# TortillasAlfred/NeuralBarkCalculator

Hardware: NVIDIA B200
Metric: images/sec (higher is better)
Workload: dtype fp16

## Files before the change

include/nbc.h:

```cpp
#ifndef NBC_H_
#define NBC_H_

#include <stddef.h>
#include <stdint.h>

#ifdef __cplusplus
extern "C" {
#endif

typedef enum {
  NBC_OK = 0,
  NBC_ERR_INVALID = -1,
  NBC_ERR_CUDA = -2,
  NBC_ERR_DEVICE = -3,
  NBC_ERR_WORKSPACE = -4,
  NBC_ERR_KERNEL = -5
} nbc_status;

typedef struct nbc_plan nbc_plan;

int nbc_version(void);
const char* nbc_last_error(void);
int nbc_device_check(int device);
int64_t nbc_launch_count(void);
// ... 15 lines not shown
                size_t workspace_bytes, void* stream);

int nbc_fold_bn_pack(const float* w, const float* gamma, const float* beta, const float* mean, const float* var,
                     const float* conv_bias, float eps, int Cout, int Cin, int kh, int kw, int cin_pad, int f16,
                     void* w_packed_bf16, float* bias_out, void* stream);

typedef struct {
  int32_t N, H, W, Cin, Cout;
  int32_t kh, kw, stride, pad, dil;
  int32_t relu;
  int32_t impl;
  int32_t f16;
} nbc_conv_desc;
int nbc_conv_bf16(const nbc_conv_desc* desc, const void* x, const void* w_packed, const float* bias,
                  const void* residual, void* y, void* stream);

int nbc_conv_dual_bf16(const nbc_conv_desc* desc, const void* x, const nbc_conv_desc* desc2, const void* x2,
                       const void* w_cat, const float* bias, void* y, void* stream);

int nbc_conv_wgrad_bf16(const nbc_conv_desc* desc, const void* dz, const void* x, float* dw, void* stream);

int nbc_stem_u8(const uint8_t* img, int N, int H, int W, const float* mean3_host, const float* std3_host,
                const float* w_stem, const float* bias, void* out, void* stream);
int nbc_stem_f32(const float* x_nchw, int N, int H, int W, const float* w_stem, const float* bias, void* out,
                 void* stream);
size_t nbc_stem_tc_workspace_bytes(int N, int H, int W);
int nbc_stem_pack_weights(const float* w_stem_f32, int f16, void* w224_bf16, void* stream);
int nbc_stem_tc(const void* input, int input_kind, int N, int H, int W, const float* mean3_host,
                const float* std3_host, const void* w224_bf16, const float* bias, int f16, void* workspace,
                size_t workspace_bytes, void* out, void* stream);
// ... 106 lines not shown
```

neuralbarkcalculator_b200/_lib.py:

```python
import ctypes as C
import os

_HERE = os.path.dirname(os.path.abspath(__file__))
LIB_PATH = os.path.join(_HERE, 'libnbc.so')

c_void_p, c_int, c_i64, c_size_t, c_float = C.c_void_p, C.c_int, C.c_int64, C.c_size_t, C.c_float


class ConvDesc(C.Structure):
    _fields_ = [(n, C.c_int32) for n in ('N', 'H', 'W', 'Cin', 'Cout', 'kh', 'kw', 'stride', 'pad', 'dil', 'relu', 'impl', 'f16')]


class PlanStep(C.Structure):
    _fields_ = ([('name', C.c_char * 24)]
                + [(n, C.c_int32) for n in ('kind', 'pair', 'halo3', 'stem_halo', 'dual', 'block_n', 'kblk', 'out_bufs',
                                            'ragged_map', 'N', 'H', 'W', 'Cin', 'Cout', 'k', 'stride', 'pad', 'dil', 'relu',
                                            'H2', 'W2', 'Cin2', 'stride2', 'level')]
                + [(n, C.c_int64) for n in ('x', 'x2', 'residual', 'y', 'levels')])


SIGNATURES = {
    'nbc_version': (c_int, []),
    'nbc_last_error': (C.c_char_p, []),
    'nbc_device_check': (c_int, [c_int]),
    'nbc_launch_count': (c_i64, []),
    'nbc_preprocess_workspace_bytes': (c_size_t, [c_int, c_int]),
    'nbc_preprocess_4x_u8': (c_int, [c_void_p, c_int, c_int, c_i64, c_int, c_void_p, c_void_p, c_void_p, c_size_t, c_void_p]),
    'nbc_preprocess_4x_span_u8': (c_int, [c_void_p, c_int, c_int, c_i64, c_int, c_int, c_int, c_void_p, c_void_p, c_void_p, c_size_t,
                                          c_void_p]),
    'nbc_preprocess_4x_batch_u8': (c_int, [c_void_p, c_void_p, c_void_p, c_int, c_int, c_int, c_i64, c_int, c_void_p, c_i64, c_void_p,
                                           c_void_p, c_size_t, c_void_p]),
    'nbc_host_zero_row_span': (c_int, [c_void_p, c_int, c_i64, c_i64, c_int, c_void_p, c_void_p]),
    'nbc_preprocess_general_workspace_bytes': (c_size_t, [c_int, c_int, c_int]),
    'nbc_preprocess_general_u8': (c_int, [c_void_p, c_int, c_int, c_i64, c_int, c_int, c_void_p, c_void_p, c_void_p, c_size_t,
                                  c_void_p]),
    'nbc_trim_u8': (c_int, [c_void_p, c_int, c_int, c_void_p, c_void_p, c_void_p, c_size_t, c_void_p]),
    'nbc_fold_bn_pack': (c_int, [c_void_p] * 6 + [c_float, c_int, c_int, c_int, c_int, c_int, c_int, c_void_p, c_void_p, c_void_p]),
    'nbc_conv_bf16': (c_int, [C.POINTER(ConvDesc), c_void_p, c_void_p, c_void_p, c_void_p, c_void_p, c_void_p]),
    'nbc_conv_dual_bf16': (c_int, [C.POINTER(ConvDesc), c_void_p, C.POINTER(ConvDesc), c_void_p, c_void_p, c_void_p, c_void_p, c_void_p]),
    'nbc_conv_wgrad_bf16': (c_int, [C.POINTER(ConvDesc), c_void_p, c_void_p, c_void_p, c_void_p]),
    'nbc_stem_u8': (c_int, [c_void_p, c_int, c_int, c_int, C.POINTER(c_float), C.POINTER(c_float), c_void_p, c_void_p, c_void_p, c_void_p]),
    'nbc_stem_f32': (c_int, [c_void_p, c_int, c_int, c_int, c_void_p, c_void_p, c_void_p, c_void_p]),
    'nbc_stem_tc_workspace_bytes': (c_size_t, [c_int, c_int, c_int]),
    'nbc_stem_pack_weights': (c_int, [c_void_p, c_int, c_void_p, c_void_p]),
    'nbc_stem_tc': (c_int, [c_void_p, c_int, c_int, c_int, c_int, C.POINTER(c_float), C.POINTER(c_float), c_void_p, c_void_p,
                    c_int, c_void_p, c_size_t, c_void_p, c_void_p]),
    'nbc_maxpool3x3s2_bf16': (c_int, [c_void_p, c_int, c_int, c_int, c_int, c_int, c_void_p, c_void_p]),
    'nbc_head_1x1': (c_int, [c_void_p, c_i64, c_int, c_int, c_int, c_void_p, c_void_p, c_void_p, c_void_p]),
    'nbc_upsample_argmax': (c_int, [c_void_p, c_int, c_int, c_int, c_int, c_int, c_void_p, c_void_p]),
    'nbc_upsample_bicubic': (c_int, [c_void_p, c_int, c_int, c_int, c_int, c_int, c_int, c_void_p, c_void_p]),
    'nbc_upsample_argmax_ragged': (c_int, [c_void_p, c_int, c_int, c_int, c_int, c_int, c_void_p, c_void_p, c_void_p]),
    'nbc_heights_from_first_last': (c_int, [c_void_p, c_int, c_void_p, c_void_p]),
    'nbc_ccl_workspace_bytes': (c_size_t, [c_int, c_int, c_int]),
# ... 90 lines not shown
```

neuralbarkcalculator_b200/csrc/api.cu:

```cuda
#include <stdarg.h>

#include "common.cuh"
#include "conv.h"
#include "train.h"

namespace nbc {

static thread_local char g_err[1024] = "";
std::atomic<int64_t> g_launches{0};

void set_error(const char* fmt, ...) {
  va_list ap;
  va_start(ap, fmt);
  vsnprintf(g_err, sizeof(g_err), fmt, ap);
  va_end(ap);
}

int sm_count() {
  static int cached = 0;
  if (cached) return cached;
  int dev = 0, n = 0;
  if (cudaGetDevice(&dev) == cudaSuccess &&
      cudaDeviceGetAttribute(&n, cudaDevAttrMultiProcessorCount, dev) == cudaSuccess && n > 0)
    cached = n;
// ... 103 lines not shown
  NBC_REQUIRE((gamma != nullptr) == (beta != nullptr) && (gamma != nullptr) == (mean != nullptr) &&
                  (gamma != nullptr) == (var != nullptr),
              "nbc_fold_bn_pack: gamma/beta/mean/var must be all given or all NULL");
  NBC_REQUIRE(Cout > 0 && Cin > 0 && kh > 0 && kw > 0 && cin_pad >= Cin, "nbc_fold_bn_pack: bad shape");
  return fold_pack(w, gamma, beta, mean, var, conv_bias, eps, Cout, Cin, kh, kw, cin_pad, w_packed_bf16, nullptr,
                   bias_out, reinterpret_cast<cudaStream_t>(stream), f16 ? 1 : 0);
}

extern "C" int nbc_conv_bf16(const nbc_conv_desc* d, const void* x, const void* w_packed, const float* bias,
                             const void* residual, void* y, void* stream_) {
  cudaStream_t stream = reinterpret_cast<cudaStream_t>(stream_);
  NBC_REQUIRE(d && x && w_packed && bias && y, "nbc_conv_bf16: null pointer");
  ConvGeom g{d->N, d->H, d->W, d->Cin, d->Cout, d->kh, d->kw, d->stride, d->pad, d->dil, d->relu, d->f16 ? 1 : 0};
  NBC_REQUIRE(g.N > 0 && g.H > 0 && g.W > 0 && g.Ho() > 0 && g.Wo() > 0, "nbc_conv_bf16: bad shape");
  const bool tc_ok = conv_tc_supported(g);
  if (d->impl == 1 || (d->impl == 0 && tc_ok)) return conv_tc(g, x, w_packed, bias, residual, y, stream);
  if (d->impl == 2 || d->impl == 0) return conv_mma(g, x, w_packed, bias, residual, y, stream);
  set_error("nbc_conv_bf16: unknown impl %d", d->impl);
  return NBC_ERR_INVALID;
}

extern "C" int nbc_conv_wgrad_bf16(const nbc_conv_desc* d, const void* dz, const void* x, float* dw, void* stream_) {
  cudaStream_t stream = reinterpret_cast<cudaStream_t>(stream_);
  NBC_REQUIRE(d && dz && x && dw, "nbc_conv_wgrad_bf16: null pointer");
  NBC_REQUIRE(!d->f16, "nbc_conv_wgrad_bf16: the training path is bf16 only");
  ConvGeom g{d->N, d->H, d->W, d->Cin, d->Cout, d->kh, d->kw, d->stride, d->pad, d->dil, 0, 0};
  NBC_REQUIRE(g.N > 0 && g.H > 0 && g.W > 0 && g.Ho() > 0 && g.Wo() > 0, "nbc_conv_wgrad_bf16: bad shape");
  const bool tc_ok = wgrad_tc_supported(g);
  if (d->impl == 1 || (d->impl == 0 && tc_ok)) return wgrad_tc(g, dz, x, dw, stream);
  if (d->impl == 2 || d->impl == 0) return wgrad_mma(g, dz, x, dw, stream);
  set_error("nbc_conv_wgrad_bf16: unknown impl %d", d->impl);
  return NBC_ERR_INVALID;
}

// ... 12 lines not shown
```

neuralbarkcalculator_b200/csrc/common.cuh:

```cuda
#pragma once
#include <cuda.h>
#include <cuda_bf16.h>
#include <cuda_fp16.h>
#include <cuda_runtime.h>
#include <stdint.h>
#include <stdio.h>

#include <atomic>
#include <string>

#include "../../include/nbc.h"

namespace nbc {

void set_error(const char* fmt, ...);
extern std::atomic<int64_t> g_launches;
inline void count_launch(int n = 1) { g_launches.fetch_add(n, std::memory_order_relaxed); }

#define NBC_CUDA(expr)                                                                       \
  do {                                                                                       \
    cudaError_t _e = (expr);                                                                 \
    if (_e != cudaSuccess) {                                                                 \
      nbc::set_error("%s failed: %s (%s:%d)", #expr, cudaGetErrorString(_e), __FILE__, __LINE__); \
      return NBC_ERR_CUDA;                                                                   \
// ... 89 lines not shown
}
__device__ __forceinline__ void tma_load_2d(void* smem, const CUtensorMap* m, uint64_t* bar, int c0, int c1) {
  asm volatile(
      "cp.async.bulk.tensor.2d.shared::cluster.global.mbarrier::complete_tx::bytes [%0], [%1, {%3, %4}], [%2];" ::"r"(
          smem_u32(smem)),
      "l"(reinterpret_cast<uint64_t>(m)), "r"(smem_u32(bar)), "r"(c0), "r"(c1)
      : "memory");
}
__device__ __forceinline__ void tma_load_4d(void* smem, const CUtensorMap* m, uint64_t* bar, int c0, int c1, int c2,
                                            int c3) {
  asm volatile(
      "cp.async.bulk.tensor.4d.shared::cluster.global.mbarrier::complete_tx::bytes [%0], [%1, {%3, %4, %5, %6}], "
      "[%2];" ::"r"(smem_u32(smem)),
      "l"(reinterpret_cast<uint64_t>(m)), "r"(smem_u32(bar)), "r"(c0), "r"(c1), "r"(c2), "r"(c3)
      : "memory");
}

__device__ __forceinline__ void tma_store_4d(const CUtensorMap* m, const void* smem, int c0, int c1, int c2, int c3) {
  asm volatile("cp.async.bulk.tensor.4d.global.shared::cta.bulk_group [%0, {%2, %3, %4, %5}], [%1];" ::"l"(
                   reinterpret_cast<uint64_t>(m)),
               "r"(smem_u32(smem)), "r"(c0), "r"(c1), "r"(c2), "r"(c3)
               : "memory");
}
__device__ __forceinline__ void tma_store_commit() { asm volatile("cp.async.bulk.commit_group;" ::: "memory"); }
template <int N>
__device__ __forceinline__ void tma_store_wait_read() {
  asm volatile("cp.async.bulk.wait_group.read %0;" ::"n"(N) : "memory");
}
__device__ __forceinline__ void tma_store_wait_all() { asm volatile("cp.async.bulk.wait_group 0;" ::: "memory"); }

// ... 156 lines not shown
```

neuralbarkcalculator_b200/csrc/conv.h:

```cpp
#pragma once
#include <cuda_runtime.h>
#include <limits.h>
#include <stdint.h>
#include <string.h>

namespace nbc {

struct ConvGeom {
  int N, H, W, Cin, Cout;
  int kh, kw, stride, pad, dil;
  int relu;
  int f16 = 0;
  int Ho() const { return (H + 2 * pad - dil * (kh - 1) - 1) / stride + 1; }
  int Wo() const { return (W + 2 * pad - dil * (kw - 1) - 1) / stride + 1; }
  double flops() const { return 2.0 * N * Ho() * Wo() * (double)Cout * Cin * kh * kw; }
};

struct ConvTcPrepared {
  alignas(64) unsigned char storage[1536];
};
bool conv_tc_supported(const ConvGeom& g);
int conv_tc_prepare(const ConvGeom& g, const void* x, const void* w, const float* bias, const void* residual, void* y,
                    ConvTcPrepared* out, const int* valid_h = nullptr);
int conv_tc_prepare_dual(const ConvGeom& g, const void* x, const ConvGeom& g2, const void* x2, const void* w_cat,
                         const float* bias, void* y, ConvTcPrepared* out, const int* valid_h = nullptr);
int conv_tc_run(const ConvTcPrepared* prep, cudaStream_t stream);
struct ConvTcVariant {
  int pair, halo3, stem_halo, dual, block_n, kblk, out_bufs;
  int ragged_map;
};
void conv_tc_describe(const ConvTcPrepared* prep, ConvTcVariant* v);
int conv_tc_prepare_stem(int N, int Ho, int Wo, int Hp, int Wp, const void* padded, const void* w224, const float* bias,
                         void* y, ConvTcPrepared* out, const int* valid_h = nullptr, int f16 = 0, int relu = 1);
int conv_tc(const ConvGeom& g, const void* x, const void* w, const float* bias, const void* residual, void* y,
            cudaStream_t stream);

bool conv_mma_supported(const ConvGeom& g);
int conv_mma(const ConvGeom& g, const void* x, const void* w, const float* bias, const void* residual, void* y,
             cudaStream_t stream);

int stem_tc_pad(const void* input, int input_kind, int N, int H, int W, const float* mean3, const float* std3, void* padded,
                cudaStream_t stream, const int* valid_h, int f16 = 0);
int maxpool_ragged(const void* x, int N, int H, int W, int C, void* y, const int* valid_h, cudaStream_t stream,
                   int f16 = 0);
int head_1x1(const void* x16, int64_t pixels_per_image, int N, int Cin, const float* w3xC, const float* bias3,
             float* logits_planar, int f16, cudaStream_t stream, const int* valid_h = nullptr, int row_w = 1);
int ragged_levels(const int* heights, const int* first_last, int N, int Hc, int* levels, cudaStream_t stream);

int fold_pack(const float* w, const float* gamma, const float* beta, const float* mean, const float* var,
              const float* cb, float eps, int Cout, int Cin, int kh, int kw, int cin_pad, void* wp_bf16, float* wp_f32,
// ... 6 lines not shown
```

neuralbarkcalculator_b200/csrc/conv_tc.cu:

```cuda
#include "common.cuh"
#include "conv.h"

namespace nbc {

struct ConvTcParams {
  CUtensorMap tmA[4];
  CUtensorMap tmB;
  CUtensorMap tmOut;
  CUtensorMap tmRes;
  const float* bias;
  const __nv_bfloat16* residual;
  __nv_bfloat16* out;
  int N, Ho, Wo, Cout;
  int tw_log2, th, tw, tiles_w, tiles_h;
  int num_m_tiles, num_n_tiles;
  int n_taps, cblocks;
  int cblocks2, map2;
  int relu;
  int f16;
  const int* valid_h;
  int8_t tap_map[9];
  int16_t tap_dh[9];
  int16_t tap_dw[9];
  const uint8_t* stem_src;
// ... 547 lines not shown
    }
    __syncwarp();
  } else if (warp == 10) {
    output_role<BN, OB, RES>(p, s, walk);
  } else {
    epilogue_role<BN, OB, RES, RELU, F16>(p, s, walk);
  }
  tc_teardown<Cfg>(warp, s.tmem_base);
}

constexpr int kStemRowBytes = 2112;
constexpr int kStemStageBytes = 7 * kStemRowBytes + 64;
using StemCfg = TcLayout<6, kStemStageBytes, 7 * 64 * 64 , 64, 4, false>;
static_assert(StemCfg::kUsedBytes > 120 * 1024, "stem halo kernel: shared memory budget");

__device__ __forceinline__ void bulk_load_1d(void* smem, const void* gmem, uint32_t bytes, uint64_t* bar) {
  asm volatile("cp.async.bulk.shared::cluster.global.mbarrier::complete_tx::bytes [%0], [%1], %2, [%3];" ::"r"(smem_u32(smem)),
               "l"(reinterpret_cast<uint64_t>(gmem)), "r"(bytes), "r"(smem_u32(bar))
               : "memory");
}
__device__ __forceinline__ uint64_t umma_desc_kmajor_noswizzle(uint32_t smem_addr, uint32_t lbo_bytes, uint32_t sbo_bytes) {
  uint64_t d = 0;
  d |= (uint64_t)((smem_addr & 0x3FFFF) >> 4);
  d |= (uint64_t)(lbo_bytes >> 4) << 16;
  d |= (uint64_t)(sbo_bytes >> 4) << 32;
  d |= (uint64_t)1 << 46;
  return d;
}

template <bool RELU, bool F16>
__global__ void __launch_bounds__(kTcThreads, 1) conv_tc_stem_kernel(const __grid_constant__ ConvTcParams p) {
  using Cfg = StemCfg;
  constexpr int BN = 64;
  const int warp = __shfl_sync(0xffffffffu, (int)(threadIdx.x >> 5), 0);
  const TcShared s = tc_prologue<Cfg>(p, warp, nullptr, false);
// ... 197 lines not shown
}

static int floordiv(int a, int b) { return (a >= 0) ? a / b : -((-a + b - 1) / b); }

struct ConvTcLaunch {
  ConvTcParams p;
  int block_n;
  int kblk;
  int grid;
  int out_bufs;
  int pair;
  int stem_halo;
  int halo3;
};

static int want_pair(bool residual, int bn, int kblocks) { return (!residual && bn == 256 && kblocks >= 8) ? 1 : 0; }
static void set_grid(ConvTcLaunch* L) {
  const ConvTcParams& p = L->p;
  const int sms = sm_count();
  if (L->pair) {
    const int pairs = ((p.num_m_tiles + 1) / 2) * p.num_n_tiles;
    L->grid = 2 * (pairs < sms / 2 ? pairs : sms / 2);
  } else {
    const int total = p.num_m_tiles * p.num_n_tiles;
    L->grid = total < sms ? total : sms;
  }
}

static int encode_out_maps(ConvTcParams* p, int N, int Ho, int Wo, int Cout, const void* y, const void* residual) {
  const uint64_t eb = 2;
  int rc = encode_act_map(&p->tmOut, y, (uint64_t)Cout, (uint64_t)Wo, (uint64_t)Ho, (uint64_t)N, (uint64_t)Cout * eb,
// ... 11 lines not shown
  int best_tw = 128, best_tiles = INT32_MAX;
  for (int tw = 128; tw >= 8; tw >>= 1) {
    const int th = 128 / tw;
    const int tiles = ceil_div(Wo, tw) * ceil_div(Ho, th);
    if (tiles < best_tiles) best_tiles = tiles, best_tw = tw;
  }
  p->tw = best_tw;
  p->th = 128 / best_tw;
  p->tw_log2 = 0;
  while ((1 << p->tw_log2) < p->tw) ++p->tw_log2;
  p->tiles_w = ceil_div(Wo, p->tw);
  p->tiles_h = ceil_div(Ho, p->th);
}

static int build_launch(const ConvGeom& g, const void* x, const void* w, const float* bias, const void* residual,
                        void* y, ConvTcLaunch* L) {
  ConvTcParams& p = L->p;
  memset(&p, 0, sizeof(p));
  const int Ho = g.Ho(), Wo = g.Wo();
  choose_tile(Ho, Wo, &p);
  p.N = g.N, p.Ho = Ho, p.Wo = Wo, p.Cout = g.Cout;
  p.num_m_tiles = g.N * p.tiles_w * p.tiles_h;
  const int bn = (g.Cout % 256 == 0) ? 256 : (g.Cout % 128 == 0 ? 128 : 64);
  L->block_n = bn;
  L->kblk = 64;
  p.num_n_tiles = g.Cout / bn;
  p.n_taps = g.kh * g.kw;
  p.cblocks = g.Cin / 64;
  p.relu = g.relu;
  p.f16 = g.f16;
  p.bias = bias;
// ... 34 lines not shown
                                2ull * g.W * g.Cin * eb, (uint64_t)g.H * g.W * g.Cin * eb, p.tw, p.th);
        if (rc) return rc;
      }
    if (!used[0]) p.tmA[0] = p.tmA[p.tap_map[0]];
  }
  L->stem_halo = 0;
  L->halo3 = (g.Cin == 64 && g.Cout == 64 && g.kh == 3 && g.kw == 3 && g.stride == 1 && g.dil == 1 && g.pad == 1 &&
              residual == nullptr && p.tw == 128 && p.th == 1)
                 ? 1
                 : 0;
  if (L->halo3) {
    int rc = encode_act_map(&p.tmA[1], xb, g.Cin, g.W, g.H, g.N, (uint64_t)g.Cin * eb, (uint64_t)g.W * g.Cin * eb,
                            (uint64_t)g.H * g.W * g.Cin * eb, kHaloW, 3);
    if (rc) return rc;
  }
  L->pair = L->halo3 ? 0 : want_pair(residual != nullptr, bn, p.n_taps * p.cblocks);
  int rc = encode_weight_map(&p.tmB, w, (uint64_t)p.n_taps * g.Cin, g.Cout, L->pair ? bn / 2 : bn);
  if (rc) return rc;
  rc = encode_out_maps(&p, g.N, Ho, Wo, g.Cout, y, residual);
  if (rc) return rc;
  L->out_bufs = (residual != nullptr || p.n_taps * p.cblocks <= 8) ? 4 : 2;
  set_grid(L);
  return 0;
}

template <void (*Kernel)(ConvTcParams), int SMEM>
static int launch_tc(const ConvTcLaunch& L, cudaStream_t stream) {
  static bool attr_set = false;
  if (!attr_set) {
    NBC_CUDA(cudaFuncSetAttribute(Kernel, cudaFuncAttributeMaxDynamicSharedMemorySize, SMEM));
    attr_set = true;
// ... 24 lines not shown
struct CtaKernels {
  template <int OB, bool RES, bool RELU, bool F16>
  static int run(const ConvTcLaunch& L, cudaStream_t stream) {
    return launch_tc<conv_tc_kernel<BN, 64, OB, RES, RELU, F16>, TcCfg<BN, 64, OB>::kSmemBytes>(L, stream);
  }
};
struct StemKernels {
  template <int OB, bool RES, bool RELU, bool F16>
  static int run(const ConvTcLaunch& L, cudaStream_t stream) {
    if constexpr (OB != 4 || RES)
      return no_kernel("per-window stem", L);
    else
      return launch_tc<conv_tc_kernel<64, 32, 4, false, RELU, F16>, TcCfg<64, 32, 4>::kSmemBytes>(L, stream);
  }
};
struct PairKernels {
  template <int OB, bool RES, bool RELU, bool F16>
  static int run(const ConvTcLaunch& L, cudaStream_t stream) {
    if constexpr (RES)
      return no_kernel("CTA-pair", L);
    else
      return launch_tc<conv_tc_pair_kernel<256, OB, false, RELU, F16>, TcCfgPair<256, OB>::kSmemBytes>(L, stream);
  }
};
struct StemHaloKernels {
  template <int OB, bool RES, bool RELU, bool F16>
  static int run(const ConvTcLaunch& L, cudaStream_t stream) {
    if constexpr (RES)
      return no_kernel("stem halo", L);
    else
      return launch_tc<conv_tc_stem_kernel<RELU, F16>, StemCfg::kSmemBytes>(L, stream);
  }
};
struct Halo3Kernels {
  template <int OB, bool RES, bool RELU, bool F16>
  static int run(const ConvTcLaunch& L, cudaStream_t stream) {
    if constexpr (RES)
// ... 48 lines not shown
  int rc = encode_weight_map(&p.tmB, w224, 224, 64, 64, 32);
  if (rc) return rc;
  rc = encode_out_maps(&p, N, Ho, Wo, 64, y, nullptr);
  if (rc) return rc;
  L->out_bufs = 4;
  L->pair = 0;
  L->halo3 = 0;
  p.stem_src = reinterpret_cast<const uint8_t*>(padded);
  p.stem_hp = Hp, p.stem_wp = Wp;
  L->stem_halo = (p.tw == 128 && p.th == 1 && (reinterpret_cast<uintptr_t>(padded) & 15) == 0) ? 1 : 0;
  set_grid(L);
  return 0;
}

int conv_tc_prepare(const ConvGeom& g, const void* x, const void* w, const float* bias, const void* residual, void* y,
                    ConvTcPrepared* out, const int* valid_h) {
  static_assert(sizeof(ConvTcLaunch) <= sizeof(out->storage), "ConvTcPrepared::storage too small");
  if (!conv_tc_supported(g)) {
    set_error("conv_tc: unsupported shape Cin=%d Cout=%d k=%dx%d stride=%d", g.Cin, g.Cout, g.kh, g.kw, g.stride);
    return NBC_ERR_INVALID;
  }
  if ((reinterpret_cast<uintptr_t>(bias) & 15) != 0) {
    set_error("conv_tc: bias must be 16-byte aligned");
    return NBC_ERR_INVALID;
  }
  ConvTcLaunch* L = reinterpret_cast<ConvTcLaunch*>(out->storage);
  int rc = build_launch(g, x, w, bias, residual, y, L);
  L->p.valid_h = valid_h;
  return rc;
}

int conv_tc_prepare_dual(const ConvGeom& g, const void* x, const ConvGeom& g2, const void* x2, const void* w_cat,
                         const float* bias, void* y, ConvTcPrepared* out, const int* valid_h) {
  if (!conv_tc_supported(g) || !conv_tc_supported(g2) || g.stride != 1 || g2.kh != 1 || g2.kw != 1 || g2.pad != 0 ||
      g2.Cout != g.Cout || g2.N != g.N || g2.Ho() != g.Ho() || g2.Wo() != g.Wo()) {
    set_error("conv_tc_prepare_dual: unsupported pair (main %dx%d k%d s%d, second Cin=%d k%d s%d)", g.Cin, g.Cout, g.kh, g.stride,
              g2.Cin, g2.kh, g2.stride);
    return NBC_ERR_INVALID;
  }
  if ((reinterpret_cast<uintptr_t>(bias) & 15) != 0) {
    set_error("conv_tc: bias must be 16-byte aligned");
    return NBC_ERR_INVALID;
// ... 2 lines not shown
  int rc = build_launch(g, x, w_cat, bias, nullptr, y, L);
  if (rc) return rc;
  ConvTcParams& p = L->p;
  p.valid_h = valid_h;
  const uint64_t eb = 2;
  const char* xb = reinterpret_cast<const char*>(x2);
  p.map2 = 1;
  p.cblocks2 = g2.Cin / 64;
  if (g2.stride == 1)
    rc = encode_act_map(&p.tmA[1], xb, g2.Cin, g2.W, g2.H, g2.N, (uint64_t)g2.Cin * eb, (uint64_t)g2.W * g2.Cin * eb,
                        (uint64_t)g2.H * g2.W * g2.Cin * eb, p.tw, p.th);
  else
    rc = encode_act_map(&p.tmA[1], xb, g2.Cin, (uint64_t)(g2.W + 1) / 2, (uint64_t)(g2.H + 1) / 2, g2.N, 2ull * g2.Cin * eb,
                        2ull * g2.W * g2.Cin * eb, (uint64_t)g2.H * g2.W * g2.Cin * eb, p.tw, p.th);
  if (rc) return rc;
  L->pair = want_pair(false, L->block_n, p.n_taps * p.cblocks + p.cblocks2);
  rc = encode_weight_map(&p.tmB, w_cat, (uint64_t)p.n_taps * g.Cin + g2.Cin, g.Cout, L->pair ? L->block_n / 2 : L->block_n);
  if (rc) return rc;
  L->out_bufs = (p.n_taps * p.cblocks + p.cblocks2 <= 8) ? 4 : 2;
  set_grid(L);
  return 0;
}

int conv_tc_run(const ConvTcPrepared* prep, cudaStream_t stream) {
  const ConvTcLaunch& L = *reinterpret_cast<const ConvTcLaunch*>(prep->storage);
  if (L.stem_halo) return launch_variant<StemHaloKernels>(L, stream);
  if (L.halo3) return launch_variant<Halo3Kernels>(L, stream);
  if (L.kblk == 32) return launch_variant<StemKernels>(L, stream);
  if (L.pair) return L.block_n == 256 ? launch_variant<PairKernels>(L, stream) : no_kernel("CTA-pair", L);
  switch (L.block_n) {
    case 256: return launch_variant<CtaKernels<256>>(L, stream);
    case 128: return launch_variant<CtaKernels<128>>(L, stream);
    case 64: return launch_variant<CtaKernels<64>>(L, stream);
    default: return no_kernel("conv_tc_kernel", L);
  }
}

void conv_tc_describe(const ConvTcPrepared* prep, ConvTcVariant* v) {
  const ConvTcLaunch* L = reinterpret_cast<const ConvTcLaunch*>(prep->storage);
  v->pair = L->pair, v->halo3 = L->halo3, v->stem_halo = L->stem_halo, v->dual = L->p.cblocks2 > 0;
  v->block_n = L->block_n, v->kblk = L->kblk, v->out_bufs = L->out_bufs;
  v->ragged_map = L->p.valid_h == nullptr ? -1 : (ragged_mapped(L->p) ? 1 : 0);
}

int conv_tc(const ConvGeom& g, const void* x, const void* w, const float* bias, const void* residual, void* y,
            cudaStream_t stream) {
  ConvTcPrepared prep;
  int rc = conv_tc_prepare(g, x, w, bias, residual, y, &prep);
  if (rc) return rc;
  return conv_tc_run(&prep, stream);
}

}
```

neuralbarkcalculator_b200/csrc/head.cu:

```cuda
#include "common.cuh"
#include "cubic.cuh"

namespace nbc {

template <int kIters>
__global__ void __launch_bounds__(256) head1x1_kernel(const __nv_bfloat16* __restrict__ x, int P, int N, int Cin,
                                                      const float* __restrict__ w, const float* __restrict__ bias,
                                                      float* __restrict__ logits, int f16, const int* __restrict__ valid_h,
                                                      int row_w) {
  const int lane = threadIdx.x & 31;
  const int warp_global = (int)((blockIdx.x * blockDim.x + threadIdx.x) >> 5);
  const int nwarps = (int)((gridDim.x * blockDim.x) >> 5);
  const int M = N * P;
  const float b0 = __ldg(bias), b1 = __ldg(bias + 1), b2 = __ldg(bias + 2);
  float wr[kIters][3][8];
#pragma unroll
  for (int it = 0; it < kIters; ++it)
#pragma unroll
    for (int k = 0; k < 3; ++k)
#pragma unroll
      for (int e = 0; e < 8; ++e) wr[it][k][e] = __ldg(w + k * Cin + it * 256 + lane * 8 + e);
  constexpr int kPix = 4;
  for (int m0 = warp_global; m0 < M; m0 += nwarps * kPix) {
    uint4 v[kPix][kIters];
    bool on[kPix];
#pragma unroll
    for (int j = 0; j < kPix; ++j) {
      const int m = m0 + j * nwarps;
      on[j] = m < M;
      if (on[j] && valid_h != nullptr) {
        const int img = m / P;
        on[j] = (m - img * P) / row_w < __ldg(valid_h + img);
      }
      if (on[j]) {
        const __nv_bfloat16* xr = x + (int64_t)m * Cin + lane * 8;
#pragma unroll
        for (int it = 0; it < kIters; ++it) v[j][it] = __ldg(reinterpret_cast<const uint4*>(xr + it * 256));
      }
    }
#pragma unroll
    for (int j = 0; j < kPix; ++j) {
      if (!on[j]) continue;
      const int m = m0 + j * nwarps;
      float a0 = 0.f, a1 = 0.f, a2 = 0.f;
#pragma unroll
      for (int it = 0; it < kIters; ++it) {
        const uint32_t u[4] = {v[j][it].x, v[j][it].y, v[j][it].z, v[j][it].w};
#pragma unroll
        for (int k = 0; k < 4; ++k) {
          const float f0 = lo16(u[k], f16), f1 = hi16(u[k], f16);
          a0 = fmaf(f0, wr[it][0][2 * k], a0), a0 = fmaf(f1, wr[it][0][2 * k + 1], a0);
          a1 = fmaf(f0, wr[it][1][2 * k], a1), a1 = fmaf(f1, wr[it][1][2 * k + 1], a1);
          a2 = fmaf(f0, wr[it][2][2 * k], a2), a2 = fmaf(f1, wr[it][2][2 * k + 1], a2);
        }
      }
#pragma unroll
      for (int o = 16; o > 0; o >>= 1) {
        a0 += __shfl_xor_sync(0xffffffffu, a0, o);
        a1 += __shfl_xor_sync(0xffffffffu, a1, o);
        a2 += __shfl_xor_sync(0xffffffffu, a2, o);
      }
      if (lane == 0) {
        const int img = m / P, pix = m - img * P;
        float* o = logits + (int64_t)img * 3 * P + pix;
        o[0] = a0 + b0;
        o[P] = a1 + b1;
        o[2 * P] = a2 + b2;
      }
    }
  }
}

__device__ __forceinline__ float cubic_sample(const float* __restrict__ plane, int w, const int (&iy)[4],
                                              const float (&wy)[4], const int (&ix)[4], const float (&wx)[4]) {
  float out = 0.f;
#pragma unroll
  for (int i = 0; i < 4; ++i) {
    const float* r = plane + (int64_t)iy[i] * w;
    float inner = __fmul_rn(__ldg(r + ix[0]), wx[0]);
    inner = __fadd_rn(inner, __fmul_rn(__ldg(r + ix[1]), wx[1]));
    inner = __fadd_rn(inner, __fmul_rn(__ldg(r + ix[2]), wx[2]));
    inner = __fadd_rn(inner, __fmul_rn(__ldg(r + ix[3]), wx[3]));
    const float term = __fmul_rn(inner, wy[i]);
    out = (i == 0) ? term : __fadd_rn(out, term);
// ... 110 lines not shown
  return 0;
}

extern "C" int nbc_upsample_argmax_ragged(const float* logits, int N, int hc, int w, int Hc, int W, const int32_t* heights,
                                          uint8_t* mask, void* stream) {
  NBC_REQUIRE(logits && heights && mask, "nbc_upsample_argmax_ragged: null pointer");
  NBC_REQUIRE(N > 0 && hc > 0 && w > 0 && Hc > 0 && W > 0 && Hc <= 65535 && N <= 65535, "nbc_upsample_argmax_ragged: bad shape");
  dim3 grid(ceil_div(W, 256), ceil_div(Hc, kK3Rows), N);
  upsample_argmax_rows_kernel<<<grid, 256, 0, reinterpret_cast<cudaStream_t>(stream)>>>(logits, hc, w, Hc, W, 0,
                                                                                         (float)w / (float)W, heights, mask);
  NBC_CHECK_LAUNCH();
  return 0;
}

namespace nbc {
int head_1x1(const void* x_bf16, int64_t pixels_per_image, int N, int Cin, const float* w3xC, const float* bias3,
             float* logits_planar, int f16, cudaStream_t stream, const int* valid_h, int row_w) {
  NBC_REQUIRE(x_bf16 && w3xC && bias3 && logits_planar, "nbc_head_1x1: null pointer");
  NBC_REQUIRE((Cin == 256 || Cin == 512 || Cin == 1024) && N > 0 && pixels_per_image > 0,
              "nbc_head_1x1: Cin must be 256, 512 or 1024 (got %d)", Cin);
  const int64_t M = (int64_t)N * pixels_per_image;
  NBC_REQUIRE(M < (1ll << 31) - (1 << 24), "nbc_head_1x1: N * pixels_per_image must be < 2^31");
  const int64_t want = ceil_div64(M, 8 * 4);
  const int blocks = (int)(want < 148 * 8 ? (want < 1 ? 1 : want) : 148 * 8);
  const __nv_bfloat16* xb = reinterpret_cast<const __nv_bfloat16*>(x_bf16);
  if (Cin == 256)
    head1x1_kernel<1><<<blocks, 256, 0, stream>>>(xb, (int)pixels_per_image, N, Cin, w3xC, bias3, logits_planar, f16, valid_h, row_w);
  else if (Cin == 512)
    head1x1_kernel<2><<<blocks, 256, 0, stream>>>(xb, (int)pixels_per_image, N, Cin, w3xC, bias3, logits_planar, f16, valid_h, row_w);
  else
    head1x1_kernel<4><<<blocks, 256, 0, stream>>>(xb, (int)pixels_per_image, N, Cin, w3xC, bias3, logits_planar, f16, valid_h, row_w);
  NBC_CHECK_LAUNCH();
  return 0;
}
}

extern "C" int nbc_head_1x1(const void* x_bf16, int64_t pixels_per_image, int N, int Cin, int f16, const float* w3xC,
                            const float* bias3, float* logits_planar, void* stream) {
  return head_1x1(x_bf16, pixels_per_image, N, Cin, w3xC, bias3, logits_planar, f16 ? 1 : 0,
                  reinterpret_cast<cudaStream_t>(stream), nullptr, 1);
}

static int upsample_common(const float* logits, int N, int C, int h, int w, int H, int W, uint8_t* mask, float* out,
                           cudaStream_t stream) {
  NBC_REQUIRE(logits && (mask || out), "nbc_upsample: null pointer");
  NBC_REQUIRE(N > 0 && C > 0 && h > 0 && w > 0 && H > 0 && W > 0 && H <= 65535 && N <= 65535, "nbc_upsample: bad shape");
  const float sy = (float)h / (float)H, sx = (float)w / (float)W;
  dim3 grid(ceil_div(W, 256), H, N);
// ... 23 lines not shown
```

neuralbarkcalculator_b200/ops.py:

```python
import ctypes as C

import torch

from . import _lib


def _stream(device=None):
    return C.c_void_p(torch.cuda.current_stream(device).cuda_stream)


def _dev(t, name='tensor'):
    if not isinstance(t, torch.Tensor) or not t.is_cuda:
        raise RuntimeError('%s must be a CUDA tensor: neuralbarkcalculator_b200 has no CPU path' % name)
    _lib.require_device(t.device.index if t.device.index is not None else torch.cuda.current_device())
    return t


def _ptr(t):
    return C.c_void_p(t.data_ptr()) if t is not None else C.c_void_p(0)


def _contig(t, dtype, name):
    _dev(t, name)
    if t.dtype != dtype:
# ... 103 lines not shown
    Cout, Cin, kh, kw = weight.shape
    cin_pad = Cin if cin_pad is None else cin_pad
    g = b = m = v = None
    if bn is not None:
        g, b, m, v = [_contig(t, torch.float32, 'bn') for t in bn]
    cb = _contig(conv_bias, torch.float32, 'conv_bias') if conv_bias is not None else None
    with torch.cuda.device(weight.device):
        wp = torch.empty((Cout, kh, kw, cin_pad), dtype=dtype, device=weight.device)
        bias = torch.empty(Cout, dtype=torch.float32, device=weight.device)
        _lib.check(lib.nbc_fold_bn_pack(_ptr(weight), _ptr(g), _ptr(b), _ptr(m), _ptr(v), _ptr(cb), eps, Cout, Cin, kh, kw,
                                        cin_pad, 1 if dtype == torch.float16 else 0, _ptr(wp), _ptr(bias),
                                        _stream(weight.device)), 'nbc_fold_bn_pack')
    return wp, bias


def conv_bf16(x, w_packed, bias, stride=1, pad=0, dil=1, relu=False, residual=None, impl=0):
    lib = _lib.load()
    x, f16 = _half(x, 'x')
    w_packed = _contig(w_packed, x.dtype, 'w_packed')
    bias = _contig(bias, torch.float32, 'bias')
    N, H, W, Cin = x.shape
    Cout, kh, kw, cin2 = w_packed.shape
    if cin2 != Cin:
        raise RuntimeError('conv_bf16: channel mismatch %d vs %d' % (Cin, cin2))
    Ho = (H + 2 * pad - dil * (kh - 1) - 1) // stride + 1
    Wo = (W + 2 * pad - dil * (kw - 1) - 1) // stride + 1
    if residual is not None:
        residual = _contig(residual, x.dtype, 'residual')
        if tuple(residual.shape) != (N, Ho, Wo, Cout):
            raise RuntimeError('conv_bf16: residual shape mismatch')
    with torch.cuda.device(x.device):
        y = torch.empty((N, Ho, Wo, Cout), dtype=x.dtype, device=x.device)
        d = _lib.ConvDesc(N, H, W, Cin, Cout, kh, kw, stride, pad, dil, 1 if relu else 0, impl, f16)
        _lib.check(lib.nbc_conv_bf16(C.byref(d), _ptr(x), _ptr(w_packed), _ptr(bias), _ptr(residual), _ptr(y),
                                     _stream(x.device)), 'nbc_conv_bf16')
    return y


def conv_dual_bf16(x, w, x2, w2, bias, stride2=1, relu=True):
    lib = _lib.load()
    x, f16 = _half(x, 'x')
    x2 = _contig(x2, x.dtype, 'x2')
    w, w2 = _contig(w, x.dtype, 'w'), _contig(w2, x.dtype, 'w2')
    bias = _contig(bias, torch.float32, 'bias')
    N, H, W, C1 = x.shape
    _, H2, W2, C2 = x2.shape
    Cout = w.shape[0]
    w_cat = torch.cat([w.reshape(Cout, C1), w2.reshape(Cout, C2)], dim=1).contiguous()
    with torch.cuda.device(x.device):
        y = torch.empty((N, H, W, Cout), dtype=x.dtype, device=x.device)
# ... 368 lines not shown
```

Measured before the change: 1404.

## Pipeline head 1x1 with bulk async loads and allow CTA-pair for residual+relu convs

Rewrites the 1x1 head kernel so each warp streams pixel rows into a shared-memory ring through cp.async.bulk with mbarriers, overlapping loads with FMA work and batching shuffle reductions across pixels. It also enables the CTA-pair conv kernel for residual convolutions that use ReLU, and adds a ragged conv entry point plus an impl flag that disables pairing. The head now needs 16-byte aligned input and a large dynamic shared-memory allocation with one block per SM. Residual pair kernels run with fewer pipeline stages.

After: 1407 (median of 6 runs). About the same (+0.2%).

```diff
diff --git a/include/nbc.h b/include/nbc.h
--- a/include/nbc.h
+++ b/include/nbc.h
@@ -53,6 +53,9 @@
 } nbc_conv_desc;
 int nbc_conv_bf16(const nbc_conv_desc* desc, const void* x, const void* w_packed, const float* bias,
                   const void* residual, void* y, void* stream);
+
+int nbc_conv_ragged_bf16(const nbc_conv_desc* desc, const void* x, const void* w_packed, const float* bias,
+                         const void* residual, const int32_t* valid_h, void* y, void* stream);
 
 int nbc_conv_dual_bf16(const nbc_conv_desc* desc, const void* x, const nbc_conv_desc* desc2, const void* x2,
                        const void* w_cat, const float* bias, void* y, void* stream);
diff --git a/neuralbarkcalculator_b200/_lib.py b/neuralbarkcalculator_b200/_lib.py
--- a/neuralbarkcalculator_b200/_lib.py
+++ b/neuralbarkcalculator_b200/_lib.py
@@ -37,6 +37,7 @@
     'nbc_trim_u8': (c_int, [c_void_p, c_int, c_int, c_void_p, c_void_p, c_void_p, c_size_t, c_void_p]),
     'nbc_fold_bn_pack': (c_int, [c_void_p] * 6 + [c_float, c_int, c_int, c_int, c_int, c_int, c_int, c_void_p, c_void_p, c_void_p]),
     'nbc_conv_bf16': (c_int, [C.POINTER(ConvDesc), c_void_p, c_void_p, c_void_p, c_void_p, c_void_p, c_void_p]),
+    'nbc_conv_ragged_bf16': (c_int, [C.POINTER(ConvDesc), c_void_p, c_void_p, c_void_p, c_void_p, c_void_p, c_void_p, c_void_p]),
     'nbc_conv_dual_bf16': (c_int, [C.POINTER(ConvDesc), c_void_p, C.POINTER(ConvDesc), c_void_p, c_void_p, c_void_p, c_void_p, c_void_p]),
     'nbc_conv_wgrad_bf16': (c_int, [C.POINTER(ConvDesc), c_void_p, c_void_p, c_void_p, c_void_p]),
     'nbc_stem_u8': (c_int, [c_void_p, c_int, c_int, c_int, C.POINTER(c_float), C.POINTER(c_float), c_void_p, c_void_p, c_void_p, c_void_p]),
diff --git a/neuralbarkcalculator_b200/csrc/api.cu b/neuralbarkcalculator_b200/csrc/api.cu
--- a/neuralbarkcalculator_b200/csrc/api.cu
+++ b/neuralbarkcalculator_b200/csrc/api.cu
@@ -141,10 +141,21 @@
   ConvGeom g{d->N, d->H, d->W, d->Cin, d->Cout, d->kh, d->kw, d->stride, d->pad, d->dil, d->relu, d->f16 ? 1 : 0};
   NBC_REQUIRE(g.N > 0 && g.H > 0 && g.W > 0 && g.Ho() > 0 && g.Wo() > 0, "nbc_conv_bf16: bad shape");
   const bool tc_ok = conv_tc_supported(g);
-  if (d->impl == 1 || (d->impl == 0 && tc_ok)) return conv_tc(g, x, w_packed, bias, residual, y, stream);
+  if (d->impl == 1 || d->impl == 3 || (d->impl == 0 && tc_ok))
+    return conv_tc(g, x, w_packed, bias, residual, y, stream, nullptr, d->impl != 3);
   if (d->impl == 2 || d->impl == 0) return conv_mma(g, x, w_packed, bias, residual, y, stream);
   set_error("nbc_conv_bf16: unknown impl %d", d->impl);
   return NBC_ERR_INVALID;
+}
+
+extern "C" int nbc_conv_ragged_bf16(const nbc_conv_desc* d, const void* x, const void* w_packed, const float* bias,
+                                    const void* residual, const int32_t* valid_h, void* y, void* stream_) {
+  cudaStream_t stream = reinterpret_cast<cudaStream_t>(stream_);
+  NBC_REQUIRE(d && x && w_packed && bias && valid_h && y, "nbc_conv_ragged_bf16: null pointer");
+  ConvGeom g{d->N, d->H, d->W, d->Cin, d->Cout, d->kh, d->kw, d->stride, d->pad, d->dil, d->relu, d->f16 ? 1 : 0};
+  NBC_REQUIRE(g.N > 0 && g.H > 0 && g.W > 0 && g.Ho() > 0 && g.Wo() > 0, "nbc_conv_ragged_bf16: bad shape");
+  NBC_REQUIRE(d->impl == 0 || d->impl == 1 || d->impl == 3, "nbc_conv_ragged_bf16: impl must be 0, 1 or 3 (got %d)", d->impl);
+  return conv_tc(g, x, w_packed, bias, residual, y, stream, valid_h, d->impl != 3);
 }
 
 extern "C" int nbc_conv_wgrad_bf16(const nbc_conv_desc* d, const void* dz, const void* x, float* dw, void* stream_) {
diff --git a/neuralbarkcalculator_b200/csrc/common.cuh b/neuralbarkcalculator_b200/csrc/common.cuh
--- a/neuralbarkcalculator_b200/csrc/common.cuh
+++ b/neuralbarkcalculator_b200/csrc/common.cuh
@@ -127,6 +127,12 @@
       "[%2];" ::"r"(smem_u32(smem)),
       "l"(reinterpret_cast<uint64_t>(m)), "r"(smem_u32(bar)), "r"(c0), "r"(c1), "r"(c2), "r"(c3)
       : "memory");
+}
+
+__device__ __forceinline__ void bulk_load_1d(void* smem, const void* gmem, uint32_t bytes, uint64_t* bar) {
+  asm volatile("cp.async.bulk.shared::cluster.global.mbarrier::complete_tx::bytes [%0], [%1], %2, [%3];" ::"r"(smem_u32(smem)),
+               "l"(reinterpret_cast<uint64_t>(gmem)), "r"(bytes), "r"(smem_u32(bar))
+               : "memory");
 }
 
 __device__ __forceinline__ void tma_store_4d(const CUtensorMap* m, const void* smem, int c0, int c1, int c2, int c3) {
diff --git a/neuralbarkcalculator_b200/csrc/conv.h b/neuralbarkcalculator_b200/csrc/conv.h
--- a/neuralbarkcalculator_b200/csrc/conv.h
+++ b/neuralbarkcalculator_b200/csrc/conv.h
@@ -21,7 +21,7 @@
 };
 bool conv_tc_supported(const ConvGeom& g);
 int conv_tc_prepare(const ConvGeom& g, const void* x, const void* w, const float* bias, const void* residual, void* y,
-                    ConvTcPrepared* out, const int* valid_h = nullptr);
+                    ConvTcPrepared* out, const int* valid_h = nullptr, bool allow_pair = true);
 int conv_tc_prepare_dual(const ConvGeom& g, const void* x, const ConvGeom& g2, const void* x2, const void* w_cat,
                          const float* bias, void* y, ConvTcPrepared* out, const int* valid_h = nullptr);
 int conv_tc_run(const ConvTcPrepared* prep, cudaStream_t stream);
@@ -33,7 +33,7 @@
 int conv_tc_prepare_stem(int N, int Ho, int Wo, int Hp, int Wp, const void* padded, const void* w224, const float* bias,
                          void* y, ConvTcPrepared* out, const int* valid_h = nullptr, int f16 = 0, int relu = 1);
 int conv_tc(const ConvGeom& g, const void* x, const void* w, const float* bias, const void* residual, void* y,
-            cudaStream_t stream);
+            cudaStream_t stream, const int* valid_h = nullptr, bool allow_pair = true);
 
 bool conv_mma_supported(const ConvGeom& g);
 int conv_mma(const ConvGeom& g, const void* x, const void* w, const float* bias, const void* residual, void* y,
diff --git a/neuralbarkcalculator_b200/csrc/conv_tc.cu b/neuralbarkcalculator_b200/csrc/conv_tc.cu
--- a/neuralbarkcalculator_b200/csrc/conv_tc.cu
+++ b/neuralbarkcalculator_b200/csrc/conv_tc.cu
@@ -585,11 +585,6 @@
 using StemCfg = TcLayout<6, kStemStageBytes, 7 * 64 * 64 , 64, 4, false>;
 static_assert(StemCfg::kUsedBytes > 120 * 1024, "stem halo kernel: shared memory budget");
 
-__device__ __forceinline__ void bulk_load_1d(void* smem, const void* gmem, uint32_t bytes, uint64_t* bar) {
-  asm volatile("cp.async.bulk.shared::cluster.global.mbarrier::complete_tx::bytes [%0], [%1], %2, [%3];" ::"r"(smem_u32(smem)),
-               "l"(reinterpret_cast<uint64_t>(gmem)), "r"(bytes), "r"(smem_u32(bar))
-               : "memory");
-}
 __device__ __forceinline__ uint64_t umma_desc_kmajor_noswizzle(uint32_t smem_addr, uint32_t lbo_bytes, uint32_t sbo_bytes) {
   uint64_t d = 0;
   d |= (uint64_t)((smem_addr & 0x3FFFF) >> 4);
@@ -817,7 +812,9 @@
   int halo3;
 };
 
-static int want_pair(bool residual, int bn, int kblocks) { return (!residual && bn == 256 && kblocks >= 8) ? 1 : 0; }
+static int want_pair(bool residual, bool relu, int bn, int kblocks) {
+  return (bn == 256 && kblocks >= 8 && (!residual || relu)) ? 1 : 0;
+}
 static void set_grid(ConvTcLaunch* L) {
   const ConvTcParams& p = L->p;
   const int sms = sm_count();
@@ -859,7 +856,7 @@
 }
 
 static int build_launch(const ConvGeom& g, const void* x, const void* w, const float* bias, const void* residual,
-                        void* y, ConvTcLaunch* L) {
+                        void* y, ConvTcLaunch* L, bool allow_pair = true) {
   ConvTcParams& p = L->p;
   memset(&p, 0, sizeof(p));
   const int Ho = g.Ho(), Wo = g.Wo();
@@ -924,7 +921,7 @@
                             (uint64_t)g.H * g.W * g.Cin * eb, kHaloW, 3);
     if (rc) return rc;
   }
-  L->pair = L->halo3 ? 0 : want_pair(residual != nullptr, bn, p.n_taps * p.cblocks);
+  L->pair = (L->halo3 || !allow_pair) ? 0 : want_pair(residual != nullptr, g.relu != 0, bn, p.n_taps * p.cblocks);
   int rc = encode_weight_map(&p.tmB, w, (uint64_t)p.n_taps * g.Cin, g.Cout, L->pair ? bn / 2 : bn);
   if (rc) return rc;
   rc = encode_out_maps(&p, g.N, Ho, Wo, g.Cout, y, residual);
@@ -979,13 +976,14 @@
       return launch_tc<conv_tc_kernel<64, 32, 4, false, RELU, F16>, TcCfg<64, 32, 4>::kSmemBytes>(L, stream);
   }
 };
+static_assert(TcCfgPair<256, 4>::kStages == 5, "residual CTA-pair kernel: shared memory budget");
 struct PairKernels {
   template <int OB, bool RES, bool RELU, bool F16>
   static int run(const ConvTcLaunch& L, cudaStream_t stream) {
-    if constexpr (RES)
+    if constexpr (RES && !RELU)
       return no_kernel("CTA-pair", L);
     else
-      return launch_tc<conv_tc_pair_kernel<256, OB, false, RELU, F16>, TcCfgPair<256, OB>::kSmemBytes>(L, stream);
+      return launch_tc<conv_tc_pair_kernel<256, OB, RES, RELU, F16>, TcCfgPair<256, OB>::kSmemBytes>(L, stream);
   }
 };
 struct StemHaloKernels {
@@ -1064,7 +1062,7 @@
 }
 
 int conv_tc_prepare(const ConvGeom& g, const void* x, const void* w, const float* bias, const void* residual, void* y,
-                    ConvTcPrepared* out, const int* valid_h) {
+                    ConvTcPrepared* out, const int* valid_h, bool allow_pair) {
   static_assert(sizeof(ConvTcLaunch) <= sizeof(out->storage), "ConvTcPrepared::storage too small");
   if (!conv_tc_supported(g)) {
     set_error("conv_tc: unsupported shape Cin=%d Cout=%d k=%dx%d stride=%d", g.Cin, g.Cout, g.kh, g.kw, g.stride);
@@ -1075,7 +1073,7 @@
     return NBC_ERR_INVALID;
   }
   ConvTcLaunch* L = reinterpret_cast<ConvTcLaunch*>(out->storage);
-  int rc = build_launch(g, x, w, bias, residual, y, L);
+  int rc = build_launch(g, x, w, bias, residual, y, L, allow_pair);
   L->p.valid_h = valid_h;
   return rc;
 }
@@ -1108,7 +1106,7 @@
     rc = encode_act_map(&p.tmA[1], xb, g2.Cin, (uint64_t)(g2.W + 1) / 2, (uint64_t)(g2.H + 1) / 2, g2.N, 2ull * g2.Cin * eb,
                         2ull * g2.W * g2.Cin * eb, (uint64_t)g2.H * g2.W * g2.Cin * eb, p.tw, p.th);
   if (rc) return rc;
-  L->pair = want_pair(false, L->block_n, p.n_taps * p.cblocks + p.cblocks2);
+  L->pair = want_pair(false, g.relu != 0, L->block_n, p.n_taps * p.cblocks + p.cblocks2);
   rc = encode_weight_map(&p.tmB, w_cat, (uint64_t)p.n_taps * g.Cin + g2.Cin, g.Cout, L->pair ? L->block_n / 2 : L->block_n);
   if (rc) return rc;
   L->out_bufs = (p.n_taps * p.cblocks + p.cblocks2 <= 8) ? 4 : 2;
@@ -1138,9 +1136,9 @@
 }
 
 int conv_tc(const ConvGeom& g, const void* x, const void* w, const float* bias, const void* residual, void* y,
-            cudaStream_t stream) {
+            cudaStream_t stream, const int* valid_h, bool allow_pair) {
   ConvTcPrepared prep;
-  int rc = conv_tc_prepare(g, x, w, bias, residual, y, &prep);
+  int rc = conv_tc_prepare(g, x, w, bias, residual, y, &prep, valid_h, allow_pair);
   if (rc) return rc;
   return conv_tc_run(&prep, stream);
 }
diff --git a/neuralbarkcalculator_b200/csrc/head.cu b/neuralbarkcalculator_b200/csrc/head.cu
--- a/neuralbarkcalculator_b200/csrc/head.cu
+++ b/neuralbarkcalculator_b200/csrc/head.cu
@@ -3,15 +3,29 @@
 
 namespace nbc {
 
+constexpr int kHeadWarps = 12, kHeadStages = 4, kHeadStageBytes = 4096;
+constexpr int kHeadSmemBytes = kHeadWarps * kHeadStages * (kHeadStageBytes + 8);
 template <int kIters>
-__global__ void __launch_bounds__(256) head1x1_kernel(const __nv_bfloat16* __restrict__ x, int P, int N, int Cin,
-                                                      const float* __restrict__ w, const float* __restrict__ bias,
-                                                      float* __restrict__ logits, int f16, const int* __restrict__ valid_h,
-                                                      int row_w) {
-  const int lane = threadIdx.x & 31;
-  const int warp_global = (int)((blockIdx.x * blockDim.x + threadIdx.x) >> 5);
-  const int nwarps = (int)((gridDim.x * blockDim.x) >> 5);
+__global__ void __launch_bounds__(kHeadWarps * 32, 1) head1x1_kernel(const __nv_bfloat16* __restrict__ x, int P, int N, int Cin,
+                                                                    const float* __restrict__ w, const float* __restrict__ bias,
+                                                                    float* __restrict__ logits, int f16,
+                                                                    const int* __restrict__ valid_h, int row_w) {
+  constexpr int kRowBytes = kIters * 512;
+  constexpr int kPix = kHeadStageBytes / kRowBytes;
+  static_assert(kPix * kHeadStages <= 32, "live bits of the ring in one word");
+  extern __shared__ __align__(128) uint8_t head_smem[];
+  const int warp = threadIdx.x >> 5, lane = threadIdx.x & 31;
+  uint8_t* ring = head_smem + warp * kHeadStages * kHeadStageBytes;
+  uint64_t* bar = reinterpret_cast<uint64_t*>(head_smem + kHeadWarps * kHeadStages * kHeadStageBytes) + warp * kHeadStages;
+  if (lane == 0) {
+    for (int i = 0; i < kHeadStages; ++i) mbar_init(&bar[i], 1);
+    fence_mbar_init();
+  }
+  __syncwarp();
   const int M = N * P;
+  const int chunks = (M + kPix - 1) / kPix;
+  const int nwarps = gridDim.x * kHeadWarps;
+  const int gw = blockIdx.x * kHeadWarps + warp;
   const float b0 = __ldg(bias), b1 = __ldg(bias + 1), b2 = __ldg(bias + 2);
   float wr[kIters][3][8];
 #pragma unroll
@@ -20,32 +34,39 @@
     for (int k = 0; k < 3; ++k)
 #pragma unroll
       for (int e = 0; e < 8; ++e) wr[it][k][e] = __ldg(w + k * Cin + it * 256 + lane * 8 + e);
-  constexpr int kPix = 4;
-  for (int m0 = warp_global; m0 < M; m0 += nwarps * kPix) {
-    uint4 v[kPix][kIters];
-    bool on[kPix];
+
+  auto issue = [&](int c, int s) -> uint32_t {
+    const int m = c * kPix + lane;
+    bool live = lane < kPix && m < M;
+    if (live && valid_h != nullptr) {
+      const int img = m / P;
+      live = (m - img * P) / row_w < __ldg(valid_h + img);
+    }
+    const uint32_t mask = __ballot_sync(0xffffffffu, live);
+    if (lane == 0) mbar_expect_tx(&bar[s], (uint32_t)__popc(mask) * kRowBytes);
+    __syncwarp();
+    if (live) bulk_load_1d(ring + s * kHeadStageBytes + lane * kRowBytes, x + (int64_t)m * Cin, kRowBytes, &bar[s]);
+    return mask;
+  };
+  uint32_t live_bits = 0;
+#pragma unroll
+  for (int s = 0; s < kHeadStages; ++s)
+    if (gw + s * nwarps < chunks) live_bits |= issue(gw + s * nwarps, s) << (s * kPix);
+
+  int s = 0;
+  uint32_t phase = 0;
+  for (int c = gw; c < chunks; c += nwarps) {
+    mbar_wait(&bar[s], phase, 900 + s);
+    const uint32_t mask = (live_bits >> (s * kPix)) & ((1u << kPix) - 1u);
+    const uint8_t* chunk = ring + s * kHeadStageBytes + lane * 16;
+    float acc[kPix][3];
 #pragma unroll
     for (int j = 0; j < kPix; ++j) {
-      const int m = m0 + j * nwarps;
-      on[j] = m < M;
-      if (on[j] && valid_h != nullptr) {
-        const int img = m / P;
-        on[j] = (m - img * P) / row_w < __ldg(valid_h + img);
-      }
-      if (on[j]) {
-        const __nv_bfloat16* xr = x + (int64_t)m * Cin + lane * 8;
-#pragma unroll
-        for (int it = 0; it < kIters; ++it) v[j][it] = __ldg(reinterpret_cast<const uint4*>(xr + it * 256));
-      }
-    }
-#pragma unroll
-    for (int j = 0; j < kPix; ++j) {
-      if (!on[j]) continue;
-      const int m = m0 + j * nwarps;
       float a0 = 0.f, a1 = 0.f, a2 = 0.f;
 #pragma unroll
       for (int it = 0; it < kIters; ++it) {
-        const uint32_t u[4] = {v[j][it].x, v[j][it].y, v[j][it].z, v[j][it].w};
+        const uint4 v = *reinterpret_cast<const uint4*>(chunk + j * kRowBytes + it * 512);
+        const uint32_t u[4] = {v.x, v.y, v.z, v.w};
 #pragma unroll
         for (int k = 0; k < 4; ++k) {
           const float f0 = lo16(u[k], f16), f1 = hi16(u[k], f16);
@@ -54,20 +75,30 @@
           a2 = fmaf(f0, wr[it][2][2 * k], a2), a2 = fmaf(f1, wr[it][2][2 * k + 1], a2);
         }
       }
-#pragma unroll
-      for (int o = 16; o > 0; o >>= 1) {
-        a0 += __shfl_xor_sync(0xffffffffu, a0, o);
-        a1 += __shfl_xor_sync(0xffffffffu, a1, o);
-        a2 += __shfl_xor_sync(0xffffffffu, a2, o);
-      }
-      if (lane == 0) {
-        const int img = m / P, pix = m - img * P;
-        float* o = logits + (int64_t)img * 3 * P + pix;
-        o[0] = a0 + b0;
-        o[P] = a1 + b1;
-        o[2 * P] = a2 + b2;
-      }
-    }
+      acc[j][0] = a0, acc[j][1] = a1, acc[j][2] = a2;
+    }
+#pragma unroll
+    for (int o = 16; o > 0; o >>= 1)
+#pragma unroll
+      for (int j = 0; j < kPix; ++j)
+#pragma unroll
+        for (int k = 0; k < 3; ++k) acc[j][k] += __shfl_xor_sync(0xffffffffu, acc[j][k], o);
+    __syncwarp();
+    const int c_next = c + kHeadStages * nwarps;
+    if (c_next < chunks) live_bits = (live_bits & ~(((1u << kPix) - 1u) << (s * kPix))) | (issue(c_next, s) << (s * kPix));
+    float r0 = acc[0][0], r1 = acc[0][1], r2 = acc[0][2];
+#pragma unroll
+    for (int j = 1; j < kPix; ++j)
+      if (lane == j) r0 = acc[j][0], r1 = acc[j][1], r2 = acc[j][2];
+    if ((mask >> lane) & 1u) {
+      const int m = c * kPix + lane;
+      const int img = m / P, pix = m - img * P;
+      float* o = logits + (int64_t)img * 3 * P + pix;
+      o[0] = r0 + b0;
+      o[P] = r1 + b1;
+      o[2 * P] = r2 + b2;
+    }
+    if (++s == kHeadStages) s = 0, phase ^= 1u;
   }
 }
 
@@ -208,6 +239,15 @@
 }
 
 namespace nbc {
+template <int kIters>
+static int launch_head(int blocks, cudaStream_t stream, const __nv_bfloat16* x, int P, int N, int Cin, const float* w,
+                       const float* bias, float* logits, int f16, const int* valid_h, int row_w) {
+  NBC_CUDA(cudaFuncSetAttribute(head1x1_kernel<kIters>, cudaFuncAttributeMaxDynamicSharedMemorySize, kHeadSmemBytes));
+  head1x1_kernel<kIters><<<blocks, kHeadWarps * 32, kHeadSmemBytes, stream>>>(x, P, N, Cin, w, bias, logits, f16, valid_h, row_w);
+  NBC_CHECK_LAUNCH();
+  return 0;
+}
+
 int head_1x1(const void* x_bf16, int64_t pixels_per_image, int N, int Cin, const float* w3xC, const float* bias3,
              float* logits_planar, int f16, cudaStream_t stream, const int* valid_h, int row_w) {
   NBC_REQUIRE(x_bf16 && w3xC && bias3 && logits_planar, "nbc_head_1x1: null pointer");
@@ -215,17 +255,16 @@
               "nbc_head_1x1: Cin must be 256, 512 or 1024 (got %d)", Cin);
   const int64_t M = (int64_t)N * pixels_per_image;
   NBC_REQUIRE(M < (1ll << 31) - (1 << 24), "nbc_head_1x1: N * pixels_per_image must be < 2^31");
-  const int64_t want = ceil_div64(M, 8 * 4);
-  const int blocks = (int)(want < 148 * 8 ? (want < 1 ? 1 : want) : 148 * 8);
+  NBC_REQUIRE((reinterpret_cast<uintptr_t>(x_bf16) & 15) == 0, "nbc_head_1x1: features must be 16-byte aligned");
+  const int64_t chunks = ceil_div64(M, 4096 / (Cin * 2));
+  const int64_t want = ceil_div64(chunks, kHeadWarps);
+  const int blocks = (int)(want < sm_count() ? want : sm_count());
   const __nv_bfloat16* xb = reinterpret_cast<const __nv_bfloat16*>(x_bf16);
   if (Cin == 256)
-    head1x1_kernel<1><<<blocks, 256, 0, stream>>>(xb, (int)pixels_per_image, N, Cin, w3xC, bias3, logits_planar, f16, valid_h, row_w);
-  else if (Cin == 512)
-    head1x1_kernel<2><<<blocks, 256, 0, stream>>>(xb, (int)pixels_per_image, N, Cin, w3xC, bias3, logits_planar, f16, valid_h, row_w);
-  else
-    head1x1_kernel<4><<<blocks, 256, 0, stream>>>(xb, (int)pixels_per_image, N, Cin, w3xC, bias3, logits_planar, f16, valid_h, row_w);
-  NBC_CHECK_LAUNCH();
-  return 0;
+    return launch_head<1>(blocks, stream, xb, (int)pixels_per_image, N, Cin, w3xC, bias3, logits_planar, f16, valid_h, row_w);
+  if (Cin == 512)
+    return launch_head<2>(blocks, stream, xb, (int)pixels_per_image, N, Cin, w3xC, bias3, logits_planar, f16, valid_h, row_w);
+  return launch_head<4>(blocks, stream, xb, (int)pixels_per_image, N, Cin, w3xC, bias3, logits_planar, f16, valid_h, row_w);
 }
 }
 
diff --git a/neuralbarkcalculator_b200/ops.py b/neuralbarkcalculator_b200/ops.py
--- a/neuralbarkcalculator_b200/ops.py
+++ b/neuralbarkcalculator_b200/ops.py
@@ -141,7 +141,7 @@
     return wp, bias
 
 
-def conv_bf16(x, w_packed, bias, stride=1, pad=0, dil=1, relu=False, residual=None, impl=0):
+def conv_bf16(x, w_packed, bias, stride=1, pad=0, dil=1, relu=False, residual=None, impl=0, valid_h=None, out=None):
     lib = _lib.load()
     x, f16 = _half(x, 'x')
     w_packed = _contig(w_packed, x.dtype, 'w_packed')
@@ -157,10 +157,22 @@
         if tuple(residual.shape) != (N, Ho, Wo, Cout):
             raise RuntimeError('conv_bf16: residual shape mismatch')
     with torch.cuda.device(x.device):
-        y = torch.empty((N, Ho, Wo, Cout), dtype=x.dtype, device=x.device)
+        if out is None:
+            y = torch.empty((N, Ho, Wo, Cout), dtype=x.dtype, device=x.device)
+        else:
+            y = _contig(out, x.dtype, 'out')
+            if tuple(y.shape) != (N, Ho, Wo, Cout):
+                raise RuntimeError('conv_bf16: out shape mismatch')
         d = _lib.ConvDesc(N, H, W, Cin, Cout, kh, kw, stride, pad, dil, 1 if relu else 0, impl, f16)
-        _lib.check(lib.nbc_conv_bf16(C.byref(d), _ptr(x), _ptr(w_packed), _ptr(bias), _ptr(residual), _ptr(y),
-                                     _stream(x.device)), 'nbc_conv_bf16')
+        if valid_h is None:
+            _lib.check(lib.nbc_conv_bf16(C.byref(d), _ptr(x), _ptr(w_packed), _ptr(bias), _ptr(residual), _ptr(y),
+                                         _stream(x.device)), 'nbc_conv_bf16')
+        else:
+            valid_h = _contig(valid_h, torch.int32, 'valid_h')
+            if tuple(valid_h.shape) != (N,):
+                raise RuntimeError('conv_bf16: valid_h must hold one row count per image')
+            _lib.check(lib.nbc_conv_ragged_bf16(C.byref(d), _ptr(x), _ptr(w_packed), _ptr(bias), _ptr(residual),
+                                                _ptr(valid_h), _ptr(y), _stream(x.device)), 'nbc_conv_ragged_bf16')
     return y
 
 
```
